# thenoobychocobo/gpt2-image-captioning

Measured on AMD Instinct MI355X. Metric: training images/sec + greedy captions/sec, GPT2-small+CLIP-B/32 at 1/2/4/8 GPU, higher is better.
Workload: dtype bf16

## Files before the change

gpt2-image-captioning_amd/csrc/gemm.hip:

```cpp
#include "gemm_tile.h"
#include "gemm_launch.h"

namespace icap {

template <typename TI>
__device__ __forceinline__ uint4 ln_chunk(const uint4 a, float mean, float rs, const float* g, const float* bt);
template <>
__device__ __forceinline__ uint4 ln_chunk<bf16_t>(const uint4 a, float mean, float rs, const float* g, const float* bt) {
  const uint32_t w[4] = {a.x, a.y, a.z, a.w};
  uint32_t o[4];
#pragma unroll
  for (int q = 0; q < 4; ++q) {
    const float v0 = (__uint_as_float(w[q] << 16) - mean) * rs * g[2 * q] + bt[2 * q];
    const float v1 = (__uint_as_float(w[q] & 0xffff0000u) - mean) * rs * g[2 * q + 1] + bt[2 * q + 1];
    o[q] = f2bf2(v0, v1);
  }
  return make_uint4(o[0], o[1], o[2], o[3]);
}
template <>
__device__ __forceinline__ uint4 ln_chunk<float>(const uint4 a, float mean, float rs, const float* g, const float* bt) {
  return make_uint4(__float_as_uint((__uint_as_float(a.x) - mean) * rs * g[0] + bt[0]),
                    __float_as_uint((__uint_as_float(a.y) - mean) * rs * g[1] + bt[1]),
                    __float_as_uint((__uint_as_float(a.z) - mean) * rs * g[2] + bt[2]),
                    __float_as_uint((__uint_as_float(a.w) - mean) * rs * g[3] + bt[3]));
}

__device__ __forceinline__ float xor16_sum(float v) {
  const auto sw = __builtin_amdgcn_permlane16_swap(__builtin_bit_cast(unsigned, v), __builtin_bit_cast(unsigned, v),
                                                   false, false);
  return __builtin_bit_cast(float, (unsigned)sw[0]) + __builtin_bit_cast(float, (unsigned)sw[1]);
}
__device__ __forceinline__ float xor32_sum(float v) {
  const auto sw = __builtin_amdgcn_permlane32_swap(__builtin_bit_cast(unsigned, v), __builtin_bit_cast(unsigned, v),
                                                   false, false);
  return __builtin_bit_cast(float, (unsigned)sw[0]) + __builtin_bit_cast(float, (unsigned)sw[1]);
}

constexpr int SK_LNK = 1280;
template <typename TI, typename TC, int NT, int MT, int SKU>
__global__ __launch_bounds__(64 * SK_WAVES) void gemm_skinny_kernel(icap_gemm_args p, uint32_t drop_thresh,
                                                                  float inv_keep) {
  constexpr int ES = sizeof(TI);
  constexpr int EPC = 16 / ES;
  constexpr int KSTEP = 4 * EPC;
  constexpr int BN = 16 * NT;
  constexpr int RLD = BN + 4;
  constexpr int HALF = SK_WAVES / 2;
  constexpr int BM = 16 * MT;
  constexpr int QPR = BN / 4;
  static_assert(BM * QPR <= 64 * SK_WAVES, "one epilogue quad per thread");
  __shared__ __attribute__((aligned(16))) float red[HALF][BM * RLD];
  __shared__ __attribute__((aligned(16))) float lngb[2 * SK_LNK];
// ... 316 lines not shown
  if (hipGetDevice(&dev) != hipSuccess || dev < 0 || dev >= 64) return 256;
  if (cus[dev] == 0) {
    int n = 0;
    if (hipDeviceGetAttribute(&n, hipDeviceAttributeMultiprocessorCount, dev) != hipSuccess || n <= 0) n = 256;
    cus[dev] = n;
  }
  return cus[dev];
}

namespace icap {
int gemm256_launch(const icap_gemm_args& p, uint32_t thr, float inv_keep, hipStream_t s);
int gemm8p_launch(const GemmPlan& pl, const icap_gemm_args& p, hipStream_t s);
}

static int gemm_acquire() { return diag_env("ICAP_FUSED_ACQUIRE", 0) == 1 ? 1 : 0; }
static int gemm_diag() { return diag_env("ICAP_GEMM_DIAG", 0) & 3; }

typedef int (*TileLauncher)(const GemmPlan&, const icap_gemm_args&, int, hipStream_t);
static TileLauncher tile_launcher(const GemmPlan& pl, const icap_gemm_args& p) {
  switch (pl.variant) {
    case V_ROLES_KOUT: return launch_tile_roles_kout;
    case V_ROLES: return launch_tile_roles;
    case V_ROLES160: return launch_tile_roles160;
    case V_ROLES96: return launch_tile_roles96;
    case V_ROLES192: return launch_tile_roles192;
    case V_R256: return launch_tile_r256;
    case V_W192: case V_W192_RING: return launch_tile_w192;
    case V_KOUT_DB: case V_KOUT_S3: return launch_tile_kout;
    case V_DB: case V_S3: case V_S4: case V_N12: case V_N13: case V_RING:
      if (pl.actk >= ACT_LNS) return launch_tile_ln;
      if (pl.actk >= ACT_FWD) return launch_tile_act;
      return p.in_dtype == ICAP_BF16 ? launch_tile_bf16 : p.in_dtype == ICAP_FP8_MX ? launch_tile_mx : launch_tile_f32;
  }
  return nullptr;
}

extern "C" const char* icap_gemm_kernel_name(const icap_gemm_args* a) {
  if (a == nullptr) return nullptr;
  GemmPlan pl;
  if (gemm_plan(*a, pl, device_cus(), plan_diag()) != ICAP_OK) return nullptr;
  return gemm_plan_kernel_name(*a, pl);
}

extern "C" int icap_gemm_plan_info(const icap_gemm_args* a, int32_t* splits, int32_t* fused) {
  ICAP_REQUIRE(a != nullptr && splits != nullptr && fused != nullptr, "icap_gemm_plan_info: null pointer");
  GemmPlan pl;
  const int rc = gemm_plan(*a, pl, device_cus(), plan_diag());
  if (rc != ICAP_OK) return rc;
  *splits = pl.skinny || pl.g256 || pl.g8p ? 1 : pl.splits;
  *fused = pl.fused ? 1 : 0;
  return ICAP_OK;
}

extern "C" int icap_gemm_group(const icap_gemm_args* a, int32_t n, void* stream) {
  ICAP_REQUIRE(a != nullptr && n >= 1 && n <= ICAP_GEMM_GROUP_MAX, "icap_gemm_group: 1 ... 8 products");
  GemmGroup g;
  g.n = 0;
  g.tstart[0] = 0;
  for (int i = 0; i < n; ++i) {
    const icap_gemm_args& p = a[i];
    icap_gemm_args q = p;
    q.split_k = 1;
    q.path = 0;
    if (const int rc = gemm_validate(q); rc != ICAP_OK) return rc;
    ICAP_REQUIRE(p.trans_ab && p.in_dtype == ICAP_BF16 && p.c_dtype == ICAP_F32,
                 "icap_gemm_group: K-outer (trans_ab) bf16 products with an fp32 C");
    ICAP_REQUIRE(p.act == ICAP_ACT_NONE && p.dact == ICAP_ACT_NONE && !p.bias && !p.resid && !p.aux && !p.ln_gamma &&
                     !p.ln_wsum && !p.ln_stats_in && !p.ln_stats_out && p.drop_p == 0.f && !p.m_dev,
                 "icap_gemm_group: plain products only (alpha, beta; no epilogue operands)");
    if (p.M == 0 || p.N == 0) continue;
    ICAP_REQUIRE(p.K > 0, "icap_gemm_group: K must be positive");
    const int k = g.n;
    g.a[k] = p;
    g.a[k].split_k = 1;
    g.a[k].tickets = nullptr;
    g.tiles_n[k] = (int)((p.N + GBN - 1) / GBN);
    g.nk[k] = (int)((p.K + 63) / 64);
    const int64_t tiles = ((p.M + GBM - 1) / GBM) * (int64_t)g.tiles_n[k];
    ICAP_REQUIRE(g.tstart[k] + tiles < (1ll << 30), "icap_gemm_group: too many tiles");
    g.tstart[k + 1] = g.tstart[k] + (int)tiles;
    ++g.n;
  }
  if (g.n == 0) return ICAP_OK;
  launch_group_kout(g, (int)device_cus(), reinterpret_cast<hipStream_t>(stream));
  return check_launch("icap_gemm_group");
}

extern "C" int icap_gemm(const icap_gemm_args* a, void* stream) {
  ICAP_REQUIRE(a != nullptr, "icap_gemm: null args");
  if (a->M == 0 || a->N == 0) return ICAP_OK;
  GemmPlan pl;
  const int prc = gemm_plan(*a, pl, device_cus(), plan_diag());
  if (prc != ICAP_OK) return prc;
  icap_gemm_args pk = *a;
  if (!pl.fused) pk.tickets = nullptr;
  const icap_gemm_args& p = pk;
  hipStream_t s = reinterpret_cast<hipStream_t>(stream);
  const uint32_t thr = pl.thr;
  const float inv_keep = pl.inv_keep;
  if (pl.skinny) {
    const dim3 sgrid(pl.grid_x, pl.grid_y), sblock(pl.block_x);
#define ICAP_SK(TI, TC, NT, U) hipLaunchKernelGGL((gemm_skinny_kernel<TI, TC, NT, 2, U>), sgrid, sblock, 0, s, p, thr, inv_keep)
#define ICAP_SKINNY_BF(TC)                                                                 \
  switch (pl.nt * 100 + pl.sku) {                                                          \
    case 103: ICAP_SK(bf16_t, TC, 1, 3); break;                                            \
    case 104: ICAP_SK(bf16_t, TC, 1, 4); break;                                            \
    case 106: ICAP_SK(bf16_t, TC, 1, 6); break;                                            \
    case 112: ICAP_SK(bf16_t, TC, 1, 12); break;                                           \
    case 203: ICAP_SK(bf16_t, TC, 2, 3); break;                                            \
    case 204: ICAP_SK(bf16_t, TC, 2, 4); break;                                            \
    case 206: ICAP_SK(bf16_t, TC, 2, 6); break;                                            \
    case 303: ICAP_SK(bf16_t, TC, 3, 3); break;                                            \
    case 304: ICAP_SK(bf16_t, TC, 3, 4); break;                                            \
    case 306: ICAP_SK(bf16_t, TC, 3, 6); break;                                            \
    case 403: ICAP_SK(bf16_t, TC, 4, 3); break;                                            \
    case 404: ICAP_SK(bf16_t, TC, 4, 4); break;                                            \
    default: ICAP_SK(bf16_t, TC, 4, 6); break;                                             \
  }
#define ICAP_SKINNY_F32(TC)                                                                \
  switch (pl.nt) {                                                                         \
    case 1: ICAP_SK(float, TC, 1, 6); break;                                               \
    case 2: ICAP_SK(float, TC, 2, 6); break;                                               \
    case 3: ICAP_SK(float, TC, 3, 6); break;                                               \
    default: ICAP_SK(float, TC, 4, 6); break;                                              \
  }
    if (p.in_dtype == ICAP_BF16) {
      if (p.c_dtype == ICAP_BF16) { ICAP_SKINNY_BF(bf16_t) } else { ICAP_SKINNY_BF(float) }
    } else {
      if (p.c_dtype == ICAP_BF16) { ICAP_SKINNY_F32(bf16_t) } else { ICAP_SKINNY_F32(float) }
    }
#undef ICAP_SKINNY_BF
#undef ICAP_SKINNY_F32
#undef ICAP_SK
    return check_launch("icap_gemm(skinny)");
  }
  if (pl.g256) return gemm256_launch(p, thr, inv_keep, s);
  if (pl.g8p) return gemm8p_launch(pl, p, s);
// ... 16 lines not shown
```

gpt2-image-captioning_amd/csrc/gemm_launch.h:

```cpp
#pragma once
#include <utility>

#include "gemm_plan.h"
#include "gemm_tile.h"

namespace icap {
int launch_tile_bf16(const GemmPlan& pl, const icap_gemm_args& p, int nks, hipStream_t s);
int launch_tile_act(const GemmPlan& pl, const icap_gemm_args& p, int nks, hipStream_t s);
int launch_tile_kout(const GemmPlan& pl, const icap_gemm_args& p, int nks, hipStream_t s);
int launch_tile_mx(const GemmPlan& pl, const icap_gemm_args& p, int nks, hipStream_t s);
int launch_tile_f32(const GemmPlan& pl, const icap_gemm_args& p, int nks, hipStream_t s);
int launch_tile_ln(const GemmPlan& pl, const icap_gemm_args& p, int nks, hipStream_t s);
int launch_tile_r256(const GemmPlan& pl, const icap_gemm_args& p, int nks, hipStream_t s);
int launch_tile_w192(const GemmPlan& pl, const icap_gemm_args& p, int nks, hipStream_t s);
int launch_tile_roles(const GemmPlan& pl, const icap_gemm_args& p, int nks, hipStream_t s);
int launch_tile_roles96(const GemmPlan& pl, const icap_gemm_args& p, int nks, hipStream_t s);
int launch_tile_roles192(const GemmPlan& pl, const icap_gemm_args& p, int nks, hipStream_t s);
int launch_tile_roles_kout(const GemmPlan& pl, const icap_gemm_args& p, int nks, hipStream_t s);
int launch_tile_roles160(const GemmPlan& pl, const icap_gemm_args& p, int nks, hipStream_t s);
constexpr int ICAP_GEMM_GROUP_MAX = 8;
struct GemmGroup {
  icap_gemm_args a[ICAP_GEMM_GROUP_MAX];
  int tiles_n[ICAP_GEMM_GROUP_MAX];
  int nk[ICAP_GEMM_GROUP_MAX];
  int tstart[ICAP_GEMM_GROUP_MAX + 1];
  int n;
};
void launch_group_kout(const GemmGroup& g, int cus, hipStream_t s);

enum KindSet : int { KINDS_PLAIN = 1, KINDS_ACT = 2, KINDS_LN = 4, KINDS_ALL = 7 };
constexpr int kind_set(int actk) { return actk >= ACT_LNS ? KINDS_LN : actk >= ACT_FWD ? KINDS_ACT : KINDS_PLAIN; }

template <typename TI, typename TC, int V, int KINDS, int KIND>
bool launch_tile_form(const GemmPlan& pl, const icap_gemm_args& p, int nks, hipStream_t s) {
  if constexpr ((kind_set(KIND) & KINDS) != 0 && tile_form_exists(V, dtype_of<TI>, dtype_of<TC>, KIND)) {
    if (pl.actk != KIND) return false;
    constexpr TileVariantInfo t = *tile_variant(V);
    hipLaunchKernelGGL((gemm_kernel<TI, TC, t.nst, t.minb, t.wm, t.wn, t.tm, t.tn, t.kout, KIND, t.roles>),
                       dim3(pl.grid_x, pl.grid_y), dim3(pl.block_x), 0, s, p, pl.tiles_n, pl.splits, nks, pl.thr, pl.inv_keep);
    return true;
  }
  return false;
}
template <typename TI, typename TC, int V, int KINDS, int... I>
bool launch_tile_kinds(const GemmPlan& pl, const icap_gemm_args& p, int nks, hipStream_t s, std::integer_sequence<int, I...>) {
  return (launch_tile_form<TI, TC, V, KINDS, epi_kind_at(I)>(pl, p, nks, s) || ...);
}
template <typename TI, int KINDS, int... V>
int launch_tile_forms(const GemmPlan& pl, const icap_gemm_args& p, int nks, hipStream_t s) {
  constexpr auto kinds = std::make_integer_sequence<int, N_EPI_KINDS>();
  const bool c16 = p.c_dtype == ICAP_BF16;
  const bool done = ((pl.variant == V && (c16 ? launch_tile_kinds<TI, bf16_t, V, KINDS>(pl, p, nks, s, kinds)
                                              : launch_tile_kinds<TI, float, V, KINDS>(pl, p, nks, s, kinds))) || ...);
  return done ? ICAP_OK : gemm_no_instantiation(pl);
}

}
```

gpt2-image-captioning_amd/csrc/gemm_plan.cpp:

```cpp
#include "gemm_plan.h"

#include <cstdio>

namespace icap {

PlanDiag plan_diag() {
  PlanDiag d;
  d.var_heavy = diag_env("ICAP_VAR_HEAVY", d.var_heavy);
  d.var_act = diag_env("ICAP_VAR_ACT", d.var_act);
  d.var_light = diag_env("ICAP_VAR_LIGHT", d.var_light);
  d.fused_s = diag_env("ICAP_FUSED_S", d.fused_s);
  d.fused_nst = diag_env("ICAP_FUSED_NST", d.fused_nst);
  if (const int v = diag_env("ICAP_FUSED_MINK", 0); v >= 2) d.fused_mink = v;
  d.kskew = diag_env("ICAP_KSKEW", d.kskew);
  d.kout_fused = diag_env("ICAP_KOUT_FUSED", 0) == 1;
  d.spec_act = diag_env("ICAP_SPEC_ACT", 1) != 0;
  d.force_tile = diag_env("ICAP_FORCE_TILE", d.force_tile);
  d.w192r = diag_env("ICAP_W192R", d.w192r);
  return d;
}

static bool al16(const void* ptr) { return (reinterpret_cast<uintptr_t>(ptr) & 15) == 0; }
static int64_t cdiv(int64_t a, int64_t b) { return (a + b - 1) / b; }
static bool plain(const icap_gemm_args& p) { return p.act == ICAP_ACT_NONE && p.dact == ICAP_ACT_NONE; }
// ... 345 lines not shown
  pl.thr = p.drop_p > 0.f ? drop_threshold(p.drop_p) : 0u;
  pl.inv_keep = p.drop_p > 0.f ? 1.f / (1.f - p.drop_p) : 1.f;
  const PlanCtx c{p, diag, cus};
  if (p.M == 0 || p.N == 0) {
    pl.nk_split = (int)c.nk;
    return ICAP_OK;
  }
  int rc;
  if ((rc = plan_skinny(c, pl)) != PASS) return rc;
  if ((rc = plan_g256(c, pl)) != PASS) return rc;
  if ((rc = plan_g8p(c, pl)) != PASS) return rc;
  if ((rc = plan_roles_kout(c, pl)) != PASS) return rc;
  TileSplit ts;
  if ((rc = plan_tile_split(c, ts)) != ICAP_OK) return rc;
  if ((rc = plan_roles(c, pl)) != PASS) return rc;
  if ((rc = plan_r256(c, ts, pl)) != PASS) return rc;
  if ((rc = plan_w192(c, ts, pl)) != PASS) return rc;
  return plan_tile128(c, ts, pl);
}

int gemm_plan_skew(const icap_gemm_args& p, const GemmPlan& pl, const PlanDiag& diag) {
  const TileVariantInfo* t = tile_variant(pl.variant);
  if (t == nullptr || t->natural_k()) return 0;
  if (p.path == 1 || p.path >= 6 || p.in_dtype == ICAP_FP8_MX || pl.nk_split > 64) return 0;
  return diag.kskew > 0 && diag.kskew < 256 ? diag.kskew : 0;
}

const char* gemm_plan_kernel_name(const icap_gemm_args& a, const GemmPlan& pl) {
  static thread_local char buf[160];
  const char* ti = a.in_dtype == ICAP_BF16 ? "unsigned short" : a.in_dtype == ICAP_FP8_MX ? "icap::fp8_t" : "float";
  const char* tc = a.c_dtype == ICAP_BF16 ? "unsigned short" : "float";
  if (pl.g256) {
    snprintf(buf, sizeof buf, "icap::gemm256_kernel<%s>", tc);
  } else if (pl.g8p) {
    snprintf(buf, sizeof buf, "icap::gemm8p_kernel<%s, %d, %d>", tc, pl.g8p, pl.actk);
  } else if (pl.skinny) {
    snprintf(buf, sizeof buf, "icap::gemm_skinny_kernel<%s, %s, %d, 2, %d>", ti, tc, pl.nt, pl.sku);
  } else if (const TileVariantInfo* t = tile_variant(pl.variant)) {
    snprintf(buf, sizeof buf, "icap::gemm_kernel<%s, %s, %d, %d, %d, %d, %d, %d, %s, %d%s>", ti, tc, t->nst, t->minb, t->wm,
             t->wn, t->tm, t->tn, t->kout ? "true" : "false", pl.actk, t->roles ? ", true" : "");
  } else {
    return nullptr;
  }
  return buf;
}

int gemm_no_instantiation(const GemmPlan& pl) {
  set_error("icap_gemm: no instantiation of " + (pl.g8p ? "the 8-phase kernel of width " + std::to_string(pl.g8p)
                                                         : "tile variant " + std::to_string(pl.variant)) +
            " with epilogue kind " + std::to_string(pl.actk) + " for these dtypes");
  return ICAP_ERR_ARG;
}

}
```

gpt2-image-captioning_amd/csrc/gemm_plan.h:

```cpp
#pragma once
#include "gemm_consts.h"
#include "host_common.h"

namespace icap {


struct EpiCaps {
  unsigned fwd = 0, bwd = 0;
  bool ln_producer = false;
  bool ln_consumer = false;
  unsigned ln_fwd = 0;
  bool ln_any = false;
  bool f32_c_plain = true;
};
constexpr unsigned A_(int act) { return 1u << act; }
constexpr unsigned A_GN = A_(ICAP_ACT_GELU_NEW), A_QG = A_(ICAP_ACT_QUICK_GELU), A_RELU = A_(ICAP_ACT_RELU),
                   A_ERF = A_(ICAP_ACT_GELU_ERF);
constexpr unsigned IN_F32 = 1u << ICAP_F32, IN_BF16 = 1u << ICAP_BF16, IN_MX = 1u << ICAP_FP8_MX;

enum TileVariant : int {
  V_DB = 0,
  V_S3 = 4,
  V_S4 = 5,
  V_N12 = 12,
// ... 61 lines not shown
  const bool fwd = a > ACT_FWD && a <= ACT_FWD + N_ACTS, bwd = a > ACT_BWD && a <= ACT_BWD + N_ACTS;
  const bool special = bf16_rm && (c_bf16 || !c.f32_c_plain);
  if (ln == 0) return a == ACT_OFF || a == ACT_ANY || (special && ((fwd && (c.fwd & A_(a - ACT_FWD))) || (bwd && (c.bwd & A_(a - ACT_BWD)))));
  if (!special) return false;
  if (ln == ACT_LNS) return c.ln_producer && a == ACT_OFF;
  if (ln == ACT_LNF) return c.ln_consumer && (a == ACT_OFF || (a == ACT_ANY && c.ln_any) || (fwd && (c.ln_fwd & A_(a - ACT_FWD))));
  return false;
}
constexpr bool tile_form_exists(int v, int in_dtype, int c_dtype, int actk) {
  const TileVariantInfo* t = tile_variant(v);
  if (t == nullptr || in_dtype < ICAP_F32 || in_dtype > ICAP_FP8_MX || !(t->in >> in_dtype & 1)) return false;
  if (c_dtype != ICAP_F32 && c_dtype != ICAP_BF16) return false;
  return epi_kind_exists(t->epi, in_dtype == ICAP_BF16 && !t->kout, c_dtype == ICAP_BF16, actk);
}
constexpr bool g8p_form_exists(int bn, int c_dtype, int actk) {
  return (bn == G8P_WIDTHS[0] || bn == G8P_WIDTHS[1]) && (c_dtype == ICAP_F32 || c_dtype == ICAP_BF16) &&
         epi_kind_exists(G8P_EPI, true, c_dtype == ICAP_BF16, actk);
}

struct GemmPlan {
  bool skinny = false;
  bool g256 = false;
  int g8p = 0;
  int nt = 1;
  int sku = 3;
  int variant = V_DB;
  int splits = 1, nk_split = 0, tiles_n = 0;
  bool fused = false;
  int actk = ACT_ANY;
  unsigned grid_x = 1, grid_y = 1, block_x = 1;
  uint32_t thr = 0;
  float inv_keep = 1.f;
};

struct PlanDiag {
  int var_heavy = V_S3, var_act = V_S3, var_light = V_S3;
  int fused_s = 0;
  int fused_nst = 0;
  int fused_mink = 24;
  int kskew = 1;
  bool kout_fused = false;
  bool spec_act = true;
  int force_tile = -1;
  int w192r = 4;
};
PlanDiag plan_diag();

int gemm_validate(const icap_gemm_args& p);
int gemm_plan(const icap_gemm_args& p, GemmPlan& pl, int cus, const PlanDiag& diag = PlanDiag());
int gemm_plan_skew(const icap_gemm_args& p, const GemmPlan& pl, const PlanDiag& diag = PlanDiag());
const char* gemm_plan_kernel_name(const icap_gemm_args& a, const GemmPlan& pl);
int gemm_no_instantiation(const GemmPlan& pl);

}
```

gpt2-image-captioning_amd/csrc/gemm_tile.h:

```cpp
#pragma once
#include "gemm_common.h"

#ifdef ICAP_STAMPS
#define ICAP_STAMP(i, v)                                                                                         \
  do {                                                                                                         \
    if (p.diag_stamps && threadIdx.x == 0) p.diag_stamps[(int64_t)blockIdx.x * 8 + (i)] = (uint64_t)(v);       \
  } while (0)
#define ICAP_NOW() __builtin_amdgcn_s_memrealtime()
#else
#define ICAP_STAMP(i, v) do {} while (0)
#define ICAP_NOW() 0ull
#endif

namespace icap {

__device__ __forceinline__ int kout_swz(int r) { return ((r & 3) << 2) | ((r >> 2) & 3); }
__device__ __forceinline__ int kout_off(int r, int ch) { return r * 256 + ((ch ^ kout_swz(r)) << 4); }
typedef short kv4s_t __attribute__((ext_vector_type(4)));
typedef __attribute__((address_space(3))) kv4s_t* kout_lds_ptr;
__device__ __forceinline__ uint4 kout_frag(const char* img, int r0, int c0, int lane) {
  const int g = lane >> 4, q = (lane >> 2) & 3, pp = lane & 3;
  const int ch = (c0 >> 3) + (pp >> 1), half = (pp & 1) * 8;
  const int kb = 8 * (g & 1) + 4 * (g >> 1);
  const char* a0 = img + kout_off(r0 + kb + q, ch) + half;
  const char* a1 = img + kout_off(r0 + 16 + kb + q, ch) + half;
  const kv4s_t lo = __builtin_amdgcn_ds_read_tr16_b64_v4i16((kout_lds_ptr)(a0));
  const kv4s_t hi = __builtin_amdgcn_ds_read_tr16_b64_v4i16((kout_lds_ptr)(a1));
  uint4 r;
  r.x = (uint32_t)(uint16_t)lo[0] | ((uint32_t)(uint16_t)lo[1] << 16);
  r.y = (uint32_t)(uint16_t)lo[2] | ((uint32_t)(uint16_t)lo[3] << 16);
  r.z = (uint32_t)(uint16_t)hi[0] | ((uint32_t)(uint16_t)hi[1] << 16);
  r.w = (uint32_t)(uint16_t)hi[2] | ((uint32_t)(uint16_t)hi[3] << 16);
  return r;
}

typedef uint32_t frag_u32x4_t __attribute__((ext_vector_type(4)));
template <int I, int N, int BASE>
struct lds_frags {
  static __device__ __forceinline__ void run(frag_u32x4_t* f, uint32_t a) {
    if constexpr (I < N) {
      asm volatile("ds_read_b128 %0, %1 offset:%2" : "=v"(f[I]) : "v"(a), "n"(BASE + I * 2048));
      lds_frags<I + 1, N, BASE>::run(f, a);
    }
  }
};

constexpr int roles_prefetch_groups(int nh, int rows_per_pass, int nhalf) {
  for (int g = 1; g < nh; ++g)
    if (nh % g == 0 && (nh / g) * rows_per_pass / nhalf <= 4) return g;
  return nh;
}
constexpr bool roles_hoist_fits(int tm, int tn) { return 4 * tm * tn + 8 * (tm + tn) <= 192; }

template <typename TI, typename TC, int NST, int MINB, int WM, int WN, int TM, int TN, bool KOUT = false, int ACT = ACT_ANY,
          bool ROLES = false>
__device__ __forceinline__ void gemm_body(icap_gemm_args p, int tiles_n, int splits, int nk_split, uint32_t drop_thresh,
                                          float inv_keep, const int bid, const int tiles_m, const int64_t Mv) {
  static_assert(!KOUT || (sizeof(TI) == 2 && 16 * WM * TM == 128 && 16 * WN * TN == 128),
                "K-outer operands: bf16, 128 x 128 tiles");
  static_assert(!ROLES || (sizeof(TI) == 2 && MINB == 1 &&
                            ((WM == 2 && WN == 2 && NST >= 3 && (!KOUT || (TM == 4 && TN == 4))) ||
                             (!KOUT && WM * WN == 8 && NST >= 2))),
                "roles: bf16 operands, 4 MFMA waves on a ring of >= 3 stages (K-outer: 128 x 128 tiles) or 8 on >= 2 "
                "(row-major), one block per CU");
  constexpr bool MX = sizeof(TI) == 1;
  constexpr int AK = ACT & 0xFF;
  constexpr int LNX = ACT >> 8;
  static_assert(!MX || (!KOUT && TM == 4 && TN == 4 && WM == 2 && WN == 2), "MX fp8: 128 x 128 tiles of 4 waves");
  constexpr int NW = WM * WN;
  constexpr int BM = 16 * WM * TM, BN = 16 * WN * TN;
  constexpr int STB = (BM + BN) * GROWB;
  constexpr int EPR = (NST >= 2 && (16 * TM) % 32 == 0) ? 32 : 16;
  constexpr int ELD = 16 * TN + 4;
  static_assert(NW * EPR * ELD * 4 <= NST * STB, "epilogue staging must fit the stage buffers");
  static_assert(BM % (8 * NW) == 0 && BN % (8 * NW) == 0, "each wave stages whole 8-row DMA pieces");
  constexpr int APW = BM / (8 * NW), BPW = BN / (8 * NW);
  __shared__ __attribute__((aligned(16))) char smem[NST * STB + (LNX == 2 ? 8 * BM : 0)];
  constexpr int ES = sizeof(TI);
  constexpr int EPC = 16 / ES;
  constexpr int BKE = GROWB / ES;

  int tid = threadIdx.x;
  if constexpr (ROLES) asm volatile("" : "+v"(tid));
  const int lane = tid & 63;
  const int wave = tid >> 6;
  const int wm = wave / WN, wn = wave - wm * WN;

  const int64_t M = p.M, N = p.N, K = p.K;
  const int tiles_mv = p.m_dev ? (int)((Mv + BM - 1) / BM) : tiles_m;
  const int nwg = tiles_mv * tiles_n * splits;
  if (bid >= nwg) return;
  const int xcd = bid & 7, q = nwg >> 3, r = nwg & 7;
  const int wgid = (xcd < r ? xcd * (q + 1) : r * (q + 1) + (xcd - r) * q) + (bid >> 3);
  const int tiles = tiles_mv * tiles_n;
  const int split = wgid / tiles, tile = wgid - split * tiles;
  const int tm = tile / tiles_n, tn = tile - tm * tiles_n;
  const int64_t m0 = (int64_t)tm * BM, n0 = (int64_t)tn * BN;
  if (m0 >= Mv) return;
  ICAP_STAMP(1, ICAP_NOW());
  const char* Ab = reinterpret_cast<const char*>(p.A) + (KOUT ? m0 : m0 * p.lda) * ES;
  const char* Bb = reinterpret_cast<const char*>(p.B) + (KOUT ? n0 : n0 * p.ldb) * ES;
  const int64_t mrows = Mv - m0 < BM ? Mv - m0 : BM;
  const int64_t nrows = N - n0 < BN ? N - n0 : BN;
  const int diag = (nk_split >> 28) & 3;
  const bool acq = (nk_split >> 30) & 1;
  const __amdgpu_buffer_rsrc_t ra_rsrc = make_rsrc(
      Ab, (diag & 1) ? 0 : (uint64_t)(KOUT ? (K - 1) * p.lda + ((mrows + 7) & ~7ll) : (mrows - 1) * p.lda + K) * ES);
  const __amdgpu_buffer_rsrc_t rb_rsrc = make_rsrc(
      Bb, (diag & 2) ? 0 : (uint64_t)(KOUT ? (K - 1) * p.ldb + ((nrows + 7) & ~7ll) : (nrows - 1) * p.ldb + K) * ES);
  const int lrow = lane >> 3;
  const int lchunk = ((lane & 7) ^ lrow) * EPC;
  uint32_t a_off[APW], b_off[BPW];
  if constexpr (KOUT) {
    const int krow = lane >> 4;
#pragma unroll
    for (int i = 0; i < APW; ++i) {
      const int row = (wave * APW + i) * 4 + krow;
// ... 173 lines not shown
    const int64_t col = n0 + ewn * 16 * TN + ec;
#pragma unroll
    for (int e = 0; e < H_EW; ++e) h_bias[e] = 0.f;
    if (whole && p.bias && p.dact == ICAP_ACT_NONE) {
#pragma unroll
      for (int e = 0; e < H_EW; ++e) h_bias[e] = (col + e < N) ? p.bias[col + e] : 0.f;
    }
    if constexpr (LNX == 2) {
#pragma unroll
      for (int e = 0; e < H_EW; ++e) h_wsum[e] = (col + e < N) ? p.ln_wsum[col + e] : 0.f;
    }
    if constexpr (HOIST_PRE) {
      const bf16_t* esrc = nullptr;
      int64_t eld = 0;
      if (whole) {
        if (AK >= ACT_BWD) {
          esrc = reinterpret_cast<const bf16_t*>(p.dact_src);
          eld = p.ld_dact;
        } else if (p.resid) {
          esrc = reinterpret_cast<const bf16_t*>(p.resid);
          eld = p.ldr;
        }
      }
      const bool want_pre = esrc != nullptr && (eld % H_EW) == 0 && (reinterpret_cast<uintptr_t>(esrc) & 15) == 0 &&
                            (p.ldc % H_EW) == 0 && (reinterpret_cast<uintptr_t>(p.C) & 15) == 0;
      if (want_pre && col + H_EW <= N) {
        const int64_t rb = m0 + ewm * 16 * TM + er;
#pragma unroll
        for (int i = 0; i < H_NEP; ++i) {
          if ((i % (EPR / H_RPI)) % H_NHALF != half) continue;
          const int64_t r0 = rb + (int64_t)i * H_RPI;
          const int64_t row = r0 < Mv ? r0 : Mv - 1;
          h_pre[i / H_NHALF] = *reinterpret_cast<const uint4*>(esrc + row * eld + col);
        }
      }
    }
    __builtin_amdgcn_sched_barrier(0);
  };

  if constexpr (ROLES) {
    constexpr int NLW = 4;
    constexpr int P = (BM + BN) / (8 * NLW);
    constexpr int PA = BM / (8 * NLW);
    static_assert((BM + BN) % (8 * NLW) == 0 && BM % (8 * NLW) == 0 && (NST - 2) * P < 64, "roles: stage split");
    const uint32_t sbase = (uint32_t)reinterpret_cast<uintptr_t>(smem);
    if constexpr (HOIST) hoist_operands();
    if (wave >= NW) {
      const int lw = wave - NW;
      uint32_t voff[P];
#pragma unroll
      for (int i = 0; i < P; ++i) {
        const int q = i * NLW + lw;
        if constexpr (KOUT) {
          const int krow = (i < PA ? q : q - BM / 8) * 4 + (lane >> 4);
          voff[i] = (uint32_t)((int64_t)krow * (i < PA ? p.lda : p.ldb) + (((lane & 15) ^ kout_swz(krow)) << 3)) * ES;
        } else {
          const int row = (i < PA ? q : q - BM / 8) * 8 + lrow;
          voff[i] = (uint32_t)((int64_t)row * (i < PA ? p.lda : p.ldb) + lchunk) * ES;
        }
      }
      auto issue = [&](int kt, int slot) __attribute__((always_inline)) {
        const bool live = kt < nk;
        const int64_t k0 = live ? kbase + kstep(kt) : 0;
        if constexpr (KOUT) {
          const uint32_t ka = (uint32_t)(k0 * p.lda * ES), kb2 = (uint32_t)(k0 * p.ldb * ES);
#pragma unroll
          for (int i = 0; i < P; ++i) {
            const uint32_t lds = __builtin_amdgcn_readfirstlane(sbase + (uint32_t)(slot * STB + (i * NLW + lw) * 1024));
            dma16a(i < PA ? ra_rsrc : rb_rsrc, lds, live ? voff[i] + (i < PA ? ka : kb2) : OOB);
          }
          return;
        }
        const uint32_t kb = (uint32_t)(k0 * ES);
        const bool kin = live && k0 + lchunk < K;
#pragma unroll
        for (int i = 0; i < P; ++i) {
          const uint32_t lds = __builtin_amdgcn_readfirstlane(sbase + (uint32_t)(slot * STB + (i * NLW + lw) * 1024));
          dma16a(i < PA ? ra_rsrc : rb_rsrc, lds, kin ? voff[i] + kb : OOB);
        }
      };
#pragma unroll
      for (int s = 0; s < NST - 1; ++s) issue(s, s);
      asm volatile("s_waitcnt vmcnt(%0)" ::"n"((NST - 2) * P) : "memory");
      __builtin_amdgcn_s_barrier();
      for (int kt = 0; kt < nk; ++kt) {
        issue(kt + NST - 1, (kt + NST - 1) % NST);
        asm volatile("s_waitcnt vmcnt(%0)" ::"n"((NST - 2) * P) : "memory");
        __builtin_amdgcn_s_barrier();
      }
      asm volatile("s_waitcnt vmcnt(0)" ::: "memory");
    } else {
    typedef frag_u32x4_t u32x4_t;
    uint32_t la[2], lb[2];
#pragma unroll
    for (int ks = 0; ks < 2; ++ks) {
      const uint32_t sw = (uint32_t)(((ks * 4 + fg) ^ (fr & 7)) << 4);
      la[ks] = (uint32_t)((wm * 16 * TM + fr) * GROWB) + sw;
      lb[ks] = (uint32_t)((wn * 16 * TN + fr) * GROWB) + sw;
    }
    u32x4_t fa0[TM], fb0[TN], fa1[TM], fb1[TN];
    auto rd = [&](u32x4_t (&fa)[TM], u32x4_t (&fb)[TN], uint32_t a, uint32_t b) __attribute__((always_inline)) {
      lds_frags<0, TM, 0>::run(fa, a);
      lds_frags<0, TN, BM * GROWB>::run(fb, b);
    };
    auto retire = [&](u32x4_t (&fa)[TM], u32x4_t (&fb)[TN]) __attribute__((always_inline)) {
      __builtin_amdgcn_sched_barrier(0);
      asm volatile("s_waitcnt lgkmcnt(0)" ::: "memory");
#pragma unroll
      for (int i = 0; i < TM; ++i) asm volatile("" : "+v"(fa[i]));
#pragma unroll
      for (int j = 0; j < TN; ++j) asm volatile("" : "+v"(fb[j]));
      __builtin_amdgcn_sched_barrier(0);
    };
    auto mm = [&](const u32x4_t (&fa)[TM], const u32x4_t (&fb)[TN]) __attribute__((always_inline)) {
#pragma unroll
      for (int i = 0; i < TM; ++i)
#pragma unroll
        for (int j = 0; j < TN; ++j)
          mfma_chunk<TI>(acc[i][j], __builtin_bit_cast(uint4, fa[i]), __builtin_bit_cast(uint4, fb[j]));
    };
    ln_prologue();
    __builtin_amdgcn_s_barrier();
    __builtin_amdgcn_sched_barrier(0);
    ICAP_STAMP(2, ICAP_NOW());
    if constexpr (KOUT) {
      auto rdk = [&](uint32_t sb, int ks, u32x4_t(&fa)[TM], u32x4_t(&fb)[TN]) __attribute__((always_inline)) {
        const char* As = smem + (sb - sbase);
#pragma unroll
        for (int i = 0; i < TM; ++i) fa[i] = __builtin_bit_cast(u32x4_t, kout_frag(As, ks * 32, wm * 16 * TM + i * 16, lane));
#pragma unroll
        for (int j = 0; j < TN; ++j)
          fb[j] = __builtin_bit_cast(u32x4_t, kout_frag(As + BM * GROWB, ks * 32, wn * 16 * TN + j * 16, lane));
      };
      rdk(sbase, 0, fa0, fb0);
      for (int kt = 0; kt < nk; ++kt) {
        const uint32_t sb = sbase + (uint32_t)((kt % NST) * STB);
        retire(fa0, fb0);
        rdk(sb, 1, fa1, fb1);
        mm(fa0, fb0);
        retire(fa1, fb1);
        __builtin_amdgcn_s_barrier();
        __builtin_amdgcn_sched_barrier(0);
        if (kt + 1 < nk) rdk(sbase + (uint32_t)(((kt + 1) % NST) * STB), 0, fa0, fb0);
        mm(fa1, fb1);
        __builtin_amdgcn_sched_barrier(0);
      }
    } else if constexpr (NW == 8) {
      for (int kt = 0; kt < nk; ++kt) {
        const uint32_t sb = sbase + (uint32_t)((kt % NST) * STB);
        rd(fa0, fb0, sb + la[0], sb + lb[0]);
        retire(fa0, fb0);
        mm(fa0, fb0);
        __builtin_amdgcn_sched_barrier(0);
        rd(fa0, fb0, sb + la[1], sb + lb[1]);
        retire(fa0, fb0);
        mm(fa0, fb0);
        __builtin_amdgcn_sched_barrier(0);
        __builtin_amdgcn_s_barrier();
      }
    } else {
    rd(fa0, fb0, sbase + la[0], sbase + lb[0]);
    for (int kt = 0; kt < nk; ++kt) {
      const uint32_t sb = sbase + (uint32_t)((kt % NST) * STB);
      retire(fa0, fb0);
      rd(fa1, fb1, sb + la[1], sb + lb[1]);
      mm(fa0, fb0);
      retire(fa1, fb1);
      __builtin_amdgcn_s_barrier();
      __builtin_amdgcn_sched_barrier(0);
      if (kt + 1 < nk) {
        const uint32_t sn = sbase + (uint32_t)(((kt + 1) % NST) * STB);
        rd(fa0, fb0, sn + la[0], sn + lb[0]);
      }
      mm(fa1, fb1);
      __builtin_amdgcn_sched_barrier(0);
    }
    }
    }
    __syncthreads();
  } else if constexpr (NST >= 3) {
    static_assert(!KOUT && !MX && sizeof(TI) == 2 && (TM == 4 || TM == 3) && TN == 4,
                  "ring: bf16 row-major operands, 64 x 64 or 48 x 64 per wave");
    constexpr int D = APW + BPW;
    typedef uint32_t u32x4_t __attribute__((ext_vector_type(4)));
    const uint32_t sbase = (uint32_t)reinterpret_cast<uintptr_t>(smem);
    uint32_t la[2], lb[2];
#pragma unroll
    for (int ks = 0; ks < 2; ++ks) {
      const uint32_t sw = (uint32_t)(((ks * 4 + fg) ^ (fr & 7)) << 4);
      la[ks] = (uint32_t)((wm * 16 * TM + fr) * GROWB) + sw;
      lb[ks] = (uint32_t)(BM * GROWB + (wn * 16 * TN + fr) * GROWB) + sw;
    }
#pragma unroll
    for (int s = 0; s < NST - 1; ++s)
      if (s < nk) load_stage(kbase + kstep(s), s);
    ln_prologue();
#define ICAP_RING_RD(dst, addr, off) asm volatile("ds_read_b128 %0, %1 offset:" #off : "=v"(dst) : "v"(addr))
    for (int kt = 0; kt < nk; ++kt) {
// ... 45 lines not shown
                     : "+v"(fa1[0]), "+v"(fa1[1]), "+v"(fa1[2]), "+v"(fb1[0]), "+v"(fb1[1]), "+v"(fb1[2]), "+v"(fb1[3]));
      __builtin_amdgcn_sched_barrier(0);
      if constexpr (NW > 4) __builtin_amdgcn_s_setprio(1);
#pragma unroll
      for (int i = 0; i < TM; ++i)
#pragma unroll
        for (int j = 0; j < 4; ++j)
          mfma_chunk<TI>(acc[i][j], __builtin_bit_cast(uint4, fa1[i]), __builtin_bit_cast(uint4, fb1[j]));
      if constexpr (NW > 4) __builtin_amdgcn_s_setprio(0);
    }
#undef ICAP_RING_RD
    __builtin_amdgcn_sched_barrier(0);
    __syncthreads();
  } else if (NST == 2) {
    load_stage(kbase + kstep(0), 0);
    load_scales(kt0, sca_cur, scb_cur);
    ln_prologue();
    asm volatile("s_waitcnt vmcnt(0)" ::: "memory");
    __syncthreads();
    ICAP_STAMP(2, ICAP_NOW());
    for (int kt = 0; kt < nk; ++kt) {
      const int cur = kt & 1;
      frag_t af[KS][TM], bfr[KS][TN];
      read_frags(smem + cur * STB, af, bfr);
      if (kt + 1 < nk) {
        load_stage(kbase + kstep(kt + 1), cur ^ 1);
        load_scales(kt0 + kt + 1, sca_nxt, scb_nxt);
      }
      mfmas(af, bfr);
      __builtin_amdgcn_sched_barrier(0);
      asm volatile("s_waitcnt vmcnt(0)" ::: "memory");
      __syncthreads();
      if constexpr (MX) {
        sca_cur = sca_nxt;
        scb_cur = scb_nxt;
      }
    }
  } else {
    for (int kt = 0; kt < nk; ++kt) {
      if (kt > 0) __syncthreads();
      load_stage(kbase + kstep(kt), 0);
      load_scales(kt0 + kt, sca_cur, scb_cur);
      if (kt == 0) ln_prologue();
      asm volatile("s_waitcnt vmcnt(0)" ::: "memory");
      __syncthreads();
      if (kt == 0) ICAP_STAMP(2, ICAP_NOW());
      frag_t af[KS][TM], bfr[KS][TN];
      read_frags(smem, af, bfr);
      mfmas(af, bfr);
    }
  }

  ICAP_STAMP(3, ICAP_NOW());
  const bool fused = !ROLES && splits > 1 && p.tickets != nullptr;
  if (fused) {
    typedef uint32_t u32x4f_t __attribute__((ext_vector_type(4)));
    int* sflag = reinterpret_cast<int*>(smem);
    __syncthreads();
    int32_t* cnt = p.tickets + 2 * (int64_t)tile;
    if (tid == 0) sflag[0] = __hip_atomic_fetch_add(cnt, 1, __ATOMIC_RELAXED, __HIP_MEMORY_SCOPE_AGENT);
    __syncthreads();
    const int order = sflag[0];
    constexpr uint32_t PB = (uint32_t)NW * TM * TN * 64 * 16;
    char* pbase = reinterpret_cast<char*>(p.workspace) + (int64_t)tile * splits * PB;
    const uint32_t lofs = (uint32_t)((wave * TM * TN * 64 + lane) * 16);
    if (order < splits - 1) {
      const __amdgpu_buffer_rsrc_t rs = make_rsrc(pbase + (int64_t)split * PB, PB);
#pragma unroll
      for (int i = 0; i < TM; ++i)
#pragma unroll
        for (int j = 0; j < TN; ++j)
          __builtin_amdgcn_raw_buffer_store_b128(__builtin_bit_cast(u32x4f_t, acc[i][j]), rs,
                                                 lofs + (uint32_t)((i * TN + j) * 1024), 0, 16 );
      asm volatile("s_waitcnt vmcnt(0)" ::: "memory");
      __syncthreads();
      if (tid == 0) __hip_atomic_fetch_add(cnt + 1, 1, __ATOMIC_RELAXED, __HIP_MEMORY_SCOPE_AGENT);
      ICAP_STAMP(0, (uint64_t)split | ((uint64_t)order << 8) | ((uint64_t)tile << 32));
      ICAP_STAMP(4, ICAP_NOW());
      return;
    }
    if (tid == 0) {
      while (__hip_atomic_load(cnt + 1, __ATOMIC_RELAXED, __HIP_MEMORY_SCOPE_AGENT) < splits - 1)
        __builtin_amdgcn_s_sleep(2);
      if (acq) {
        __builtin_amdgcn_fence(__ATOMIC_ACQUIRE, "agent");
        asm volatile("s_waitcnt vmcnt(0)" ::: "memory");
      }
      __hip_atomic_store(cnt, 0, __ATOMIC_RELAXED, __HIP_MEMORY_SCOPE_AGENT);
      __hip_atomic_store(cnt + 1, 0, __ATOMIC_RELAXED, __HIP_MEMORY_SCOPE_AGENT);
    }
    __syncthreads();
    const __amdgpu_buffer_rsrc_t rs = make_rsrc(pbase, (uint64_t)PB * splits);
    constexpr int GI = (MINB >= 3 || TM % 2 != 0) ? 1 : 2;
#pragma unroll
    for (int i0 = 0; i0 < TM; i0 += GI) {
      f32x4_t v[3][GI][TN];
#pragma unroll
      for (int q = 0; q < 3; ++q) {
        if (q < splits - 1) {
          const int sq = q < split ? q : q + 1;
#pragma unroll
          for (int ii = 0; ii < GI; ++ii)
#pragma unroll
            for (int j = 0; j < TN; ++j)
              v[q][ii][j] = __builtin_bit_cast(f32x4_t, __builtin_amdgcn_raw_buffer_load_b128(
                  rs, (uint32_t)sq * PB + lofs + (uint32_t)(((i0 + ii) * TN + j) * 1024), 0, 16 ));
// ... 231 lines not shown
```

gpt2-image-captioning_amd/csrc/gemm_tile_roles_kout.hip:

```cpp
#include "gemm_launch.h"

namespace icap {

int launch_tile_roles_kout(const GemmPlan& pl, const icap_gemm_args& p, int nks, hipStream_t s) {
  return launch_tile_forms<bf16_t, KINDS_ALL, V_ROLES_KOUT>(pl, p, nks, s);
}

constexpr TileVariantInfo KG = *tile_variant(V_ROLES_KOUT);
__global__ __launch_bounds__(KG.threads(), (KG.minb * KG.threads() / 64 + 3) / 4) void gemm_group_kernel(GemmGroup g) {
  const int total = g.tstart[g.n];
  for (int b = blockIdx.x; b < total; b += gridDim.x) {
    int i = 0;
    while (i + 1 < g.n && b >= g.tstart[i + 1]) ++i;
    const icap_gemm_args p = g.a[i];
    const int tn = g.tiles_n[i];
    const int tm = (g.tstart[i + 1] - g.tstart[i]) / tn;
    gemm_body<bf16_t, float, KG.nst, KG.minb, KG.wm, KG.wn, KG.tm, KG.tn, KG.kout, ACT_OFF, KG.roles>(p, tn, 1, g.nk[i], 0u, 1.f,
                                                                                                  b - g.tstart[i], tm, p.M);
  }
}

void launch_group_kout(const GemmGroup& g, int cus, hipStream_t s) {
  const int total = g.tstart[g.n];
  hipLaunchKernelGGL(gemm_group_kernel, dim3((unsigned)(total < cus ? total : cus)), dim3(KG.threads()), 0, s, g);
}

}
```

Baseline: 14890.

## Add 128x256 split-roles tile path for grouped K-outer GEMMs with operand swap

Adds a planner for grouped K-outer GEMMs that picks a 128x256 tile kernel (768 threads, 8 MFMA waves plus loader roles) when the total tile count fits within one wave of CUs. Products whose N is at most 4 get A/B and M/N swapped and are stored transposed through a dedicated epilogue. The aim is to cut per-tile overhead and improve operand reuse for small-batch weight-gradient groups. It adds a new LDS read path and loader offsets for 256-wide B tiles, an env override, and a host check tool. The risks are LDS bank conflicts and lower occupancy on the new path.

```diff
diff --git a/gpt2-image-captioning_amd/csrc/gemm.hip b/gpt2-image-captioning_amd/csrc/gemm.hip
--- a/gpt2-image-captioning_amd/csrc/gemm.hip
+++ b/gpt2-image-captioning_amd/csrc/gemm.hip
@@ -1,3 +1,5 @@
+#include <cstdlib>
+
 #include "gemm_tile.h"
 #include "gemm_launch.h"
 
@@ -420,11 +422,19 @@
   return ICAP_OK;
 }
 
+static bool group_force128() {
+  const char* e = std::getenv("ICAP_GROUP128");
+  return e != nullptr && std::atoi(e) == 1;
+}
+
 extern "C" int icap_gemm_group(const icap_gemm_args* a, int32_t n, void* stream) {
   ICAP_REQUIRE(a != nullptr && n >= 1 && n <= ICAP_GEMM_GROUP_MAX, "icap_gemm_group: 1 ... 8 products");
+  static_assert(ICAP_GEMM_GROUP_MAX == GROUP_MAX, "the group's planner and its kernel argument hold the same count");
   GemmGroup g;
   g.n = 0;
+  g.swap = 0;
   g.tstart[0] = 0;
+  int64_t Ms[ICAP_GEMM_GROUP_MAX], Ns[ICAP_GEMM_GROUP_MAX];
   for (int i = 0; i < n; ++i) {
     const icap_gemm_args& p = a[i];
     icap_gemm_args q = p;
@@ -442,15 +452,26 @@
     g.a[k] = p;
     g.a[k].split_k = 1;
     g.a[k].tickets = nullptr;
-    g.tiles_n[k] = (int)((p.N + GBN - 1) / GBN);
-    g.nk[k] = (int)((p.K + 63) / 64);
-    const int64_t tiles = ((p.M + GBM - 1) / GBM) * (int64_t)g.tiles_n[k];
-    ICAP_REQUIRE(g.tstart[k] + tiles < (1ll << 30), "icap_gemm_group: too many tiles");
-    g.tstart[k + 1] = g.tstart[k] + (int)tiles;
+    g.nk[k] = (int)((p.K + 63) / 64) | (gemm_diag() << 28);
+    Ms[k] = p.M, Ns[k] = p.N;
     ++g.n;
   }
   if (g.n == 0) return ICAP_OK;
-  launch_group_kout(g, (int)device_cus(), reinterpret_cast<hipStream_t>(stream));
+  const int cus = (int)device_cus();
+  const GroupPlan gp = gemm_group_plan(Ms, Ns, g.n, cus, group_force128());
+  ICAP_REQUIRE(gp.total < (1ll << 30), "icap_gemm_group: too many tiles");
+  for (int k = 0; k < g.n; ++k) {
+    if (gp.big && ((gp.swap >> k) & 1)) {
+      icap_gemm_args& p = g.a[k];
+      std::swap(p.A, p.B);
+      std::swap(p.lda, p.ldb);
+      std::swap(p.M, p.N);
+    }
+    g.tiles_n[k] = gp.tiles_n[k];
+    g.tstart[k + 1] = g.tstart[k] + gp.tiles_m[k] * gp.tiles_n[k];
+  }
+  g.swap = gp.big ? gp.swap : 0u;
+  launch_group_kout(g, cus, gp.big, reinterpret_cast<hipStream_t>(stream));
   return check_launch("icap_gemm_group");
 }
 
diff --git a/gpt2-image-captioning_amd/csrc/gemm_launch.h b/gpt2-image-captioning_amd/csrc/gemm_launch.h
--- a/gpt2-image-captioning_amd/csrc/gemm_launch.h
+++ b/gpt2-image-captioning_amd/csrc/gemm_launch.h
@@ -25,8 +25,9 @@
   int nk[ICAP_GEMM_GROUP_MAX];
   int tstart[ICAP_GEMM_GROUP_MAX + 1];
   int n;
+  unsigned swap;
 };
-void launch_group_kout(const GemmGroup& g, int cus, hipStream_t s);
+void launch_group_kout(const GemmGroup& g, int cus, bool big, hipStream_t s);
 
 enum KindSet : int { KINDS_PLAIN = 1, KINDS_ACT = 2, KINDS_LN = 4, KINDS_ALL = 7 };
 constexpr int kind_set(int actk) { return actk >= ACT_LNS ? KINDS_LN : actk >= ACT_FWD ? KINDS_ACT : KINDS_PLAIN; }
diff --git a/gpt2-image-captioning_amd/csrc/gemm_plan.cpp b/gpt2-image-captioning_amd/csrc/gemm_plan.cpp
--- a/gpt2-image-captioning_amd/csrc/gemm_plan.cpp
+++ b/gpt2-image-captioning_amd/csrc/gemm_plan.cpp
@@ -421,4 +421,22 @@
   return ICAP_ERR_ARG;
 }
 
-}
+GroupPlan gemm_group_plan(const int64_t* M, const int64_t* N, int n, int cus, bool force128) {
+  GroupPlan big, small;
+  big.big = true;
+  for (int i = 0; i < n && i < GROUP_MAX; ++i) {
+    const bool sw = N[i] <= GROUP_SWAP_N;
+    const int64_t rows = sw ? N[i] : M[i], cols = sw ? M[i] : N[i];
+    const int64_t bm = cdiv(rows, GROUP_BM), bn = cdiv(cols, GROUP_BN_BIG);
+    const int64_t sm = cdiv(M[i], GBM), sn = cdiv(N[i], GBN);
+    const int64_t cap = 1ll << 30;
+    big.tiles_m[i] = (int)(bm < cap ? bm : cap), big.tiles_n[i] = (int)(bn < cap ? bn : cap);
+    small.tiles_m[i] = (int)(sm < cap ? sm : cap), small.tiles_n[i] = (int)(sn < cap ? sn : cap);
+    if (sw) big.swap |= 1u << i;
+    big.total += (bm < cap && bn < cap && bm * bn < cap) ? bm * bn : cap;
+    small.total += (sm < cap && sn < cap && sm * sn < cap) ? sm * sn : cap;
+  }
+  return (!force128 && big.total <= cus) ? big : small;
+}
+
+}
diff --git a/gpt2-image-captioning_amd/csrc/gemm_plan.h b/gpt2-image-captioning_amd/csrc/gemm_plan.h
--- a/gpt2-image-captioning_amd/csrc/gemm_plan.h
+++ b/gpt2-image-captioning_amd/csrc/gemm_plan.h
@@ -137,4 +137,13 @@
 const char* gemm_plan_kernel_name(const icap_gemm_args& a, const GemmPlan& pl);
 int gemm_no_instantiation(const GemmPlan& pl);
 
+constexpr int GROUP_MAX = 8, GROUP_BM = 128, GROUP_BN_BIG = 256, GROUP_SWAP_N = 4;
+struct GroupPlan {
+  bool big = false;
+  unsigned swap = 0;
+  int tiles_m[GROUP_MAX] = {}, tiles_n[GROUP_MAX] = {};
+  int64_t total = 0;
+};
+GroupPlan gemm_group_plan(const int64_t* M, const int64_t* N, int n, int cus, bool force128);
+
 }
diff --git a/gpt2-image-captioning_amd/csrc/gemm_tile.h b/gpt2-image-captioning_amd/csrc/gemm_tile.h
--- a/gpt2-image-captioning_amd/csrc/gemm_tile.h
+++ b/gpt2-image-captioning_amd/csrc/gemm_tile.h
@@ -15,15 +15,17 @@
 namespace icap {
 
 __device__ __forceinline__ int kout_swz(int r) { return ((r & 3) << 2) | ((r >> 2) & 3); }
-__device__ __forceinline__ int kout_off(int r, int ch) { return r * 256 + ((ch ^ kout_swz(r)) << 4); }
+template <int ROWB = 256>
+__device__ __forceinline__ int kout_off(int r, int ch) { return r * ROWB + ((ch ^ kout_swz(r)) << 4); }
 typedef short kv4s_t __attribute__((ext_vector_type(4)));
 typedef __attribute__((address_space(3))) kv4s_t* kout_lds_ptr;
+template <int ROWB = 256>
 __device__ __forceinline__ uint4 kout_frag(const char* img, int r0, int c0, int lane) {
   const int g = lane >> 4, q = (lane >> 2) & 3, pp = lane & 3;
   const int ch = (c0 >> 3) + (pp >> 1), half = (pp & 1) * 8;
   const int kb = 8 * (g & 1) + 4 * (g >> 1);
-  const char* a0 = img + kout_off(r0 + kb + q, ch) + half;
-  const char* a1 = img + kout_off(r0 + 16 + kb + q, ch) + half;
+  const char* a0 = img + kout_off<ROWB>(r0 + kb + q, ch) + half;
+  const char* a1 = img + kout_off<ROWB>(r0 + 16 + kb + q, ch) + half;
   const kv4s_t lo = __builtin_amdgcn_ds_read_tr16_b64_v4i16((kout_lds_ptr)(a0));
   const kv4s_t hi = __builtin_amdgcn_ds_read_tr16_b64_v4i16((kout_lds_ptr)(a1));
   uint4 r;
@@ -55,14 +57,17 @@
 template <typename TI, typename TC, int NST, int MINB, int WM, int WN, int TM, int TN, bool KOUT = false, int ACT = ACT_ANY,
           bool ROLES = false>
 __device__ __forceinline__ void gemm_body(icap_gemm_args p, int tiles_n, int splits, int nk_split, uint32_t drop_thresh,
-                                          float inv_keep, const int bid, const int tiles_m, const int64_t Mv) {
-  static_assert(!KOUT || (sizeof(TI) == 2 && 16 * WM * TM == 128 && 16 * WN * TN == 128),
-                "K-outer operands: bf16, 128 x 128 tiles");
+                                          float inv_keep, const int bid, const int tiles_m, const int64_t Mv,
+                                          const bool tstore = false) {
+  static_assert(!KOUT || (sizeof(TI) == 2 && 16 * WM * TM == 128 &&
+                          (16 * WN * TN == 128 || (ROLES && 16 * WN * TN == 256 && TN == 4))),
+                "K-outer operands: bf16, 128 x 128 tiles (split roles: or 128 x 256 of 8 MFMA waves)");
   static_assert(!ROLES || (sizeof(TI) == 2 && MINB == 1 &&
                             ((WM == 2 && WN == 2 && NST >= 3 && (!KOUT || (TM == 4 && TN == 4))) ||
+                             (KOUT && WM == 2 && WN == 4 && TM == 4 && TN == 4 && NST >= 3) ||
                              (!KOUT && WM * WN == 8 && NST >= 2))),
                 "roles: bf16 operands, 4 MFMA waves on a ring of >= 3 stages (K-outer: 128 x 128 tiles) or 8 on >= 2 "
-                "(row-major), one block per CU");
+                "(row-major; K-outer: 128 x 256 tiles on >= 3), one block per CU");
   constexpr bool MX = sizeof(TI) == 1;
   constexpr int AK = ACT & 0xFF;
   constexpr int LNX = ACT >> 8;
@@ -342,8 +347,14 @@
       for (int i = 0; i < P; ++i) {
         const int q = i * NLW + lw;
         if constexpr (KOUT) {
-          const int krow = (i < PA ? q : q - BM / 8) * 4 + (lane >> 4);
-          voff[i] = (uint32_t)((int64_t)krow * (i < PA ? p.lda : p.ldb) + (((lane & 15) ^ kout_swz(krow)) << 3)) * ES;
+          constexpr int BLPR = BN / 8;
+          if (i < PA || BLPR == 16) {
+            const int krow = (i < PA ? q : q - BM / 8) * 4 + (lane >> 4);
+            voff[i] = (uint32_t)((int64_t)krow * (i < PA ? p.lda : p.ldb) + (((lane & 15) ^ kout_swz(krow)) << 3)) * ES;
+          } else {
+            const int krow = (q - BM / 8) * (64 / BLPR) + lane / BLPR;
+            voff[i] = (uint32_t)((int64_t)krow * p.ldb + (((lane & (BLPR - 1)) ^ kout_swz(krow)) << 3)) * ES;
+          }
         } else {
           const int row = (i < PA ? q : q - BM / 8) * 8 + lrow;
           voff[i] = (uint32_t)((int64_t)row * (i < PA ? p.lda : p.ldb) + lchunk) * ES;
@@ -420,8 +431,46 @@
         for (int i = 0; i < TM; ++i) fa[i] = __builtin_bit_cast(u32x4_t, kout_frag(As, ks * 32, wm * 16 * TM + i * 16, lane));
 #pragma unroll
         for (int j = 0; j < TN; ++j)
-          fb[j] = __builtin_bit_cast(u32x4_t, kout_frag(As + BM * GROWB, ks * 32, wn * 16 * TN + j * 16, lane));
+          fb[j] = __builtin_bit_cast(u32x4_t, kout_frag<2 * BN>(As + BM * GROWB, ks * 32, wn * 16 * TN + j * 16, lane));
       };
+      const int kq = 8 * (fg & 1) + 4 * (fg >> 1) + ((lane >> 2) & 3);
+      uint32_t xa = (uint32_t)(((wm * 2 * TM + ((lane & 3) >> 1)) ^ kout_swz(kq)) << 4);
+      uint32_t xb = (uint32_t)(((wn * 2 * TN + ((lane & 3) >> 1)) ^ kout_swz(kq)) << 4);
+      const uint32_t ra = (uint32_t)(kq * 2 * BM + (lane & 1) * 8);
+      const uint32_t rbb = (uint32_t)(BM * GROWB + kq * 2 * BN + (lane & 1) * 8);
+      auto rdk8 = [&](uint32_t sb, int ks, u32x4_t(&fa)[TM], u32x4_t(&fb)[TN]) __attribute__((always_inline)) {
+        asm volatile("" : "+v"(xa), "+v"(xb));
+        const uint32_t ba = sb + ra + (uint32_t)(ks * 32 * 2 * BM), bb = sb + rbb + (uint32_t)(ks * 32 * 2 * BN);
+        auto frag = [&](uint32_t a0, uint32_t step16) __attribute__((always_inline)) {
+          const kv4s_t lo = __builtin_amdgcn_ds_read_tr16_b64_v4i16((kout_lds_ptr)(uintptr_t)a0);
+          const kv4s_t hi = __builtin_amdgcn_ds_read_tr16_b64_v4i16((kout_lds_ptr)(uintptr_t)(a0 + step16));
+          u32x4_t r;
+          r.x = (uint32_t)(uint16_t)lo[0] | ((uint32_t)(uint16_t)lo[1] << 16);
+          r.y = (uint32_t)(uint16_t)lo[2] | ((uint32_t)(uint16_t)lo[3] << 16);
+          r.z = (uint32_t)(uint16_t)hi[0] | ((uint32_t)(uint16_t)hi[1] << 16);
+          r.w = (uint32_t)(uint16_t)hi[2] | ((uint32_t)(uint16_t)hi[3] << 16);
+          return r;
+        };
+#pragma unroll
+        for (int i = 0; i < TM; ++i) fa[i] = frag(ba + (xa ^ (uint32_t)(i << 5)), 16 * 2 * BM);
+#pragma unroll
+        for (int j = 0; j < TN; ++j) fb[j] = frag(bb + (xb ^ (uint32_t)(j << 5)), 16 * 2 * BN);
+      };
+      if constexpr (BN == 256) {
+        rdk8(sbase, 0, fa0, fb0);
+        for (int kt = 0; kt < nk; ++kt) {
+          const uint32_t sb = sbase + (uint32_t)((kt % NST) * STB);
+          retire(fa0, fb0);
+          rdk8(sb, 1, fa1, fb1);
+          mm(fa0, fb0);
+          retire(fa1, fb1);
+          __builtin_amdgcn_s_barrier();
+          __builtin_amdgcn_sched_barrier(0);
+          if (kt + 1 < nk) rdk8(sbase + (uint32_t)(((kt + 1) % NST) * STB), 0, fa0, fb0);
+          mm(fa1, fb1);
+          __builtin_amdgcn_sched_barrier(0);
+        }
+      } else {
       rdk(sbase, 0, fa0, fb0);
       for (int kt = 0; kt < nk; ++kt) {
         const uint32_t sb = sbase + (uint32_t)((kt % NST) * STB);
@@ -434,6 +483,7 @@
         if (kt + 1 < nk) rdk(sbase + (uint32_t)(((kt + 1) % NST) * STB), 0, fa0, fb0);
         mm(fa1, fb1);
         __builtin_amdgcn_sched_barrier(0);
+      }
       }
     } else if constexpr (NW == 8) {
       for (int kt = 0; kt < nk; ++kt) {
@@ -585,6 +635,31 @@
   }
 
   ICAP_STAMP(3, ICAP_NOW());
+  if constexpr (KOUT && ROLES && BN == 256) {
+    if (tstore) {
+      if (wave < NW && wm == 0 && fg == 0) {
+        float* C = reinterpret_cast<float*>(p.C);
+#pragma unroll
+        for (int j = 0; j < TN; ++j) {
+          const int64_t c = n0 + wn * 16 * TN + j * 16 + fr;
+#pragma unroll
+          for (int v = 0; v < 4; ++v) {
+            if (m0 + v < Mv && c < N) {
+              float x[1] = {acc[0][j][v]}, a1[1];
+              const float b0[1] = {0.f};
+              epi_fwd_act<1, ACT_OFF>(p, x, b0, a1);
+              float* cp = C + c * p.ldc + (m0 + v);
+              *cp = p.beta != 0.f ? x[0] + p.beta * *cp : x[0];
+            }
+          }
+        }
+      }
+      ICAP_STAMP(0, (uint64_t)tile << 32);
+      ICAP_STAMP(4, ICAP_NOW());
+      ICAP_STAMP(5, ICAP_NOW());
+      return;
+    }
+  }
   const bool fused = !ROLES && splits > 1 && p.tickets != nullptr;
   if (fused) {
     typedef uint32_t u32x4f_t __attribute__((ext_vector_type(4)));
diff --git a/gpt2-image-captioning_amd/csrc/gemm_tile_roles_kout.hip b/gpt2-image-captioning_amd/csrc/gemm_tile_roles_kout.hip
--- a/gpt2-image-captioning_amd/csrc/gemm_tile_roles_kout.hip
+++ b/gpt2-image-captioning_amd/csrc/gemm_tile_roles_kout.hip
@@ -20,9 +20,24 @@
   }
 }
 
-void launch_group_kout(const GemmGroup& g, int cus, hipStream_t s) {
+__global__ __launch_bounds__(768, 3) void gemm_group256_kernel(GemmGroup g) {
   const int total = g.tstart[g.n];
-  hipLaunchKernelGGL(gemm_group_kernel, dim3((unsigned)(total < cus ? total : cus)), dim3(KG.threads()), 0, s, g);
+  for (int b = blockIdx.x; b < total; b += gridDim.x) {
+    int i = 0;
+    while (i + 1 < g.n && b >= g.tstart[i + 1]) ++i;
+    const icap_gemm_args p = g.a[i];
+    const int tn = g.tiles_n[i];
+    const int tm = (g.tstart[i + 1] - g.tstart[i]) / tn;
+    gemm_body<bf16_t, float, 3, 1, 2, 4, 4, 4, true, ACT_OFF, true>(p, tn, 1, g.nk[i], 0u, 1.f, b - g.tstart[i], tm, p.M,
+                                                                   (g.swap >> i) & 1u);
+  }
+}
+
+void launch_group_kout(const GemmGroup& g, int cus, bool big, hipStream_t s) {
+  const int total = g.tstart[g.n];
+  const dim3 grid((unsigned)(total < cus ? total : cus));
+  if (big) hipLaunchKernelGGL(gemm_group256_kernel, grid, dim3(768), 0, s, g);
+  else hipLaunchKernelGGL(gemm_group_kernel, grid, dim3(KG.threads()), 0, s, g);
 }
 
 }
diff --git a/gpt2-image-captioning_amd/csrc/group_check.cpp b/gpt2-image-captioning_amd/csrc/group_check.cpp
--- /dev/null
+++ b/gpt2-image-captioning_amd/csrc/group_check.cpp
@@ -0,0 +1,27 @@
+#include <cstdio>
+#include <sstream>
+#include <string>
+#include <iostream>
+
+#include "gemm_plan.h"
+
+namespace icap {
+void set_error(const std::string&) {}
+}
+using namespace icap;
+
+int main() {
+  std::string line;
+  while (std::getline(std::cin, line)) {
+    std::istringstream in(line);
+    int cus = 0, force = 0, n = 0;
+    int64_t M[GROUP_MAX], N[GROUP_MAX];
+    if (!(in >> cus >> force)) continue;
+    while (n < GROUP_MAX && (in >> M[n] >> N[n])) ++n;
+    const GroupPlan gp = gemm_group_plan(M, N, n, cus, force != 0);
+    std::printf("%s %lld %u", gp.big ? "big" : "small", (long long)gp.total, gp.swap);
+    for (int i = 0; i < n; ++i) std::printf(" %dx%d", gp.tiles_m[i], gp.tiles_n[i]);
+    std::printf("\n");
+  }
+  return 0;
+}
```

New measurement: 15090, median of 6. 1.01x the previous value.
